# daisy9542/yolo-puncture

Hardware: AMD Instinct MI355X
Metric: images/sec (higher is better)
Workload: dtype bf16

## Files before the change

include/yolop.h:

```cpp
#ifndef YOLOP_H
#define YOLOP_H

#include <stddef.h>
#include <stdint.h>

#ifdef __cplusplus
extern "C" {
#endif

#define YP_OK 0
#define YP_ERR_ARG -1
#define YP_ERR_STATE -2
#define YP_ERR_HIP -3
#define YP_ERR_WEIGHT -4

#define YP_BF16 0
#define YP_F32 1

#define YP_TASK_DETECT 0
#define YP_TASK_SEGMENT 1

#define YP_NM 32
#define YP_MAX_MASKS 480
#define YP_ID_MASKS_FRAMES_BUDGET (1ull << 30)
// ... 137 lines not shown

int yp_debug_force_conv_cfg(int cfg);
int yp_debug_op_cfg(const yp_engine* e, int i, int* cfg);
int yp_debug_last_store_form(void);
int yp_debug_max_workgroups(int n);
int yp_debug_conv_families(int* base, int* num_cfgs, int cap);
int yp_debug_ablation(int v);
int yp_debug_head_clocks(uint64_t* out8);
int yp_debug_attention(const void* qkv_dev, void* o_dev, int dtype, int B, int N, int nh, int kd, int hd, int q_stride, int q_coff, int o_stride,
                       int o_coff, int wgs, int* kernel_out, void* stream);
int yp_debug_attention_form(const void* qkv_dev, void* o_dev, int dtype, int B, int N, int nh, int kd, int hd, int q_stride, int q_coff, int o_stride,
                            int o_coff, int wgs, int form, int* kernel_out, void* stream);
int yp_debug_conv_s2(const void* x_dev, const void* w_dev, const float* bias_dev, const void* res_dev, void* y_dev, int out_f32, int B, int H,
                     int W, int Cin, int Cout, int silu, int cfg, int lds_weights, int64_t* lds_out, char* kernel_out, int kernel_cap,
                     void* stream);
int yp_debug_topk_anchors(const uint32_t* const mk_dev[3], int B, const int hw[3][2], int k, int32_t* sel_out_dev, uint32_t* thr_out_dev, void* stream);
int yp_debug_head_branch_clocks(uint64_t* out8);
int yp_debug_head_winners(yp_engine* e, int32_t* sel_host, float* box_host, float* coeff_host);
int yp_debug_contour_clocks(uint64_t* out12);
int yp_debug_pwsp_clocks(uint64_t* out32);

int yp_tuning_source(const yp_engine* e);

int yp_debug_host_selftest(yp_engine* e);
int yp_debug_graph_info(const yp_engine* e, int64_t* out6);
int yp_debug_head_positions(yp_engine* e, int64_t* out6);
int yp_debug_marker(void* stream);

int yp_set_graph(yp_engine* e, int enable);

// ... 5 lines not shown
```

yolo-puncture_amd/csrc/common.h:

```cpp
#pragma once
#include <hip/hip_runtime.h>
#include <stdint.h>
#include <atomic>
#include <cstdlib>
#include <initializer_list>
#include <string>
#include <type_traits>
#include <vector>

namespace yp {

enum DType { DT_BF16 = 0, DT_F32 = 1 };
enum Act { ACT_NONE = 0, ACT_SILU = 1, ACT_RELU = 2 };

enum OpKind {
    OP_STEM = 0,
    OP_CONV = 1,
    OP_DWCONV = 2,
    OP_POOL5 = 3,
    OP_UPSAMPLE = 4,
    OP_ATTN = 5,
    OP_HEAD = 6,
    OP_CONVT = 7,
    OP_AMAX = 9,
// ... 352 lines not shown
                           size_t rows, hipStream_t st);
hipError_t launch_anchor_max_level(const float* cls, int B, int HW, int nc, unsigned* out, hipStream_t st);

struct DwPwParams {
    const void* x; int x_stride, x_coff; int B, H, W, C; size_t x_bytes;
    const void* w_dw; const float* b_dw; int act_dw;
    const void* w_pw; int Kpad; size_t wpw_bytes; const float* b_pw; int act_pw;
    void* y; int y_stride, y_coff; size_t y_bytes; int Cout; int out_f32;
    unsigned long long* clk;
    int wide;
    const void* w3; int Kpad3; size_t w3_bytes; const float* b3; int C3;
    float* y3; int y3_stride, y3_coff; size_t y3_bytes;
    unsigned* keys;
};
bool dwpw_stream_valid(const DwPwParams& p);
hipError_t launch_dwpw_stream(const DwPwParams& p, hipStream_t st);
struct PwSpParams {
    const void* x; int x_stride, x_coff; size_t x_bytes; int B, H, W, K;
    const void* w1; const float* bias1; int act1, Kpad1, C1; size_t w1_bytes;
    void* y1; int y1_stride, y1_coff;
    const void* res1; int res1_stride, res1_coff;
    int sp;
    int sp_c0, Csp;
    const void* wd; const float* biasd; int actd;
    const void* res; int res_stride, res_coff;
    void* y2; int y2_stride, y2_coff;
    int dbg;
    int wide;
};
bool pwsp_valid(const PwSpParams& p);
// ... 76 lines not shown
```

yolo-puncture_amd/csrc/conv_dwpw.hip:

```cpp
#include "common.h"
#include <cstdio>
#include <cstdlib>
#include <vector>

namespace yp {

template <int TH, int BN, bool OUT_F32, int NW, bool TAIL = false>
__global__ __launch_bounds__(NW * 64) void conv_dwpw_kernel(const DwPwParams p, const int tiles_h, const int tiles_w, const int ntiles,
                                                       const int G) {
    constexpr int WGM = 2, WGN = NW / 2;
    constexpr int RPW = TH / NW;
    static_assert(RPW * NW == TH && RPW >= 1, "rows per wave");
    constexpr int BM = TH * 16;
    constexpr int HP = (TH + 2) * 18;
    constexpr int H_INSTR = (HP * 4 + 63) / 64;
    constexpr int LH = (H_INSTR + NW - 1) / NW;
    constexpr int HB = H_INSTR * 1024;
    constexpr int NSH = 3;
    constexpr int WM = BM / WGM, WN = BN / WGN, FM = WM / 16, FN = WN / 16;
    constexpr int S = FM * FN;
    static_assert(LH + 2 * S < 64, "vmcnt immediate");

    extern __shared__ __attribute__((aligned(1024))) unsigned char smem[];
    const int nchunk = p.C >> 5;
// ... 355 lines not shown
    if (dwpw_stream_valid(p)) return true;
    if ((p.C % 32) != 0 || p.Kpad != p.C || (p.Cout & 3) || (p.y_stride & 3) || (p.y_coff & 3)) return false;
    if (p.x_bytes >= (1ull << 31) || p.y_bytes >= (1ull << 31) || p.wpw_bytes >= (1ull << 31)) return false;
    if ((long)((p.H + 7) / 8 * 8) * ((p.W + 15) / 16 * 16) * 2 > (long)p.H * p.W * 3) return false;
    const int bn = dwpw_bn(p);
    if (bn == 0) return false;
    if ((p.Cout + bn - 1) / bn > 2) return false;
    if (dwpw_tail(p)) {
        if (p.Cout > bn || p.C < 64 || p.C3 <= 0 || p.C3 > 128 || (p.C3 & 3) || (p.y3_stride & 3) || (p.y3_coff & 3) || !p.y3 || !p.b3) return false;
        if (p.Kpad3 != (p.Cout + 31) / 32 * 32 || p.y3_bytes >= (1ull << 31) || p.w3_bytes >= (1ull << 31) || (size_t)p.B * p.H * p.W * 4 >= (1ull << 31)) return false;
    }
    return true;
}

const char* conv_dwpw_kernel_name(const DwPwParams& p) {
    if (dwpw_stream_valid(p)) return "conv_dwpw_stream_kernel";
    const int bn = dwpw_bn(p);
    if (dwpw_tail(p)) return bn == 128 ? "conv_dwpw_kernel<8,128,tail,8>" : "conv_dwpw_kernel<8,64,tail,8>";
    if (p.out_f32) return bn == 128 ? "conv_dwpw_kernel<8,128,true,8>" : "conv_dwpw_kernel<8,64,true,8>";
    return bn == 128 ? "conv_dwpw_kernel<8,128,false,8>" : "conv_dwpw_kernel<8,64,false,8>";
}

template <int BN, bool OUT_F32, bool TAIL = false>
static hipError_t launch_dwpw_t(const DwPwParams& p, hipStream_t st) {
    constexpr int TH = 8, NW = 8;
    const size_t sh = dwpw_lds(TH, BN, p.C, TAIL ? p.C3 : 0);
    const int tiles_h = (p.H + TH - 1) / TH, tiles_w = (p.W + 15) / 16, ntiles = (p.Cout + BN - 1) / BN;
    const int num_tiles = p.B * tiles_h * tiles_w;
    int G = 256 / ntiles;
    if (sh <= 80 * 1024 && NW == 4) G *= 2;
    if (G < 1) G = 1;
// ... 41 lines not shown
```

yolo-puncture_amd/csrc/conv_dwpw_stream.hip:

```cpp
#include "common.h"
#include <cstdlib>

namespace yp {

constexpr int DS_TH = 8, DS_TW = 16;
constexpr int DS_C = 128;
constexpr int DS_HP = (DS_TH + 2) * (DS_TW + 2);
constexpr int DS_PIECES = 48;
constexpr int DS_HB = DS_PIECES * 1024;
constexpr int DS_AB = DS_TH * DS_TW * 256;

template <int NW>
__global__ __launch_bounds__(NW * 64, 2) void conv_dwpw_stream_kernel(const DwPwParams p, const int tiles_h, const int tiles_w, const int num_tiles, const int G) {
    constexpr int RPW = DS_TH / NW;
    constexpr int NFW = 8 / NW;
    constexpr int NSLOT = NW == 8 ? 2 : 1;
    constexpr int NST = DS_TH * NFW;
    extern __shared__ __attribute__((aligned(1024))) unsigned char smem[];
    unsigned char* const Hs = smem;
    unsigned char* const As = smem + NSLOT * DS_HB;
    const int tid = threadIdx.x, lane = tid & 63;
    const int wave = __builtin_amdgcn_readfirstlane(tid >> 6);
    const int fr = lane & 15, fc = lane >> 4;
    const bool wide = NFW % 2 == 0 && p.wide != 0;

    const __amdgpu_buffer_rsrc_t xrs = __builtin_amdgcn_make_buffer_rsrc((void*)p.x, 0, (int)p.x_bytes, 0x00020000);
    const __amdgpu_buffer_rsrc_t wrs = __builtin_amdgcn_make_buffer_rsrc((void*)p.w_pw, 0, (int)p.wpw_bytes, 0x00020000);
    const __amdgpu_buffer_rsrc_t yrs = __builtin_amdgcn_make_buffer_rsrc((void*)p.y, 0, (int)p.y_bytes, 0x00020000);

    unsigned hyx[DS_PIECES / NW];
#pragma unroll
    for (int j = 0; j < DS_PIECES / NW; ++j) {
        const int hp = ((wave + j * NW) * 64 + lane) >> 4;
        const int hy = hp / (DS_TW + 2);
        hyx[j] = (unsigned)((hy << 8) | (hp - hy * (DS_TW + 2)));
    }
    auto issue_tile = [&](int tile, int slot) {
        int t = tile;
        const int tw = t % tiles_w; t /= tiles_w;
        const int th = t % tiles_h;
        const int b = t / tiles_h;
        const int h0 = th * DS_TH - 1, w0 = tw * DS_TW - 1;
        unsigned char* const dst = Hs + slot * DS_HB;
#pragma unroll
        for (int j = 0; j < DS_PIECES / NW; ++j) {
            const int ii = wave + j * NW;
            const int s = ii * 64 + lane;
            const int hp = s >> 4, c = s & 15;
            unsigned q = hyx[j];
            asm volatile("" : "+v"(q));
            const int hy = (int)(q >> 8), hx = (int)(q & 255u);
            const int hi = h0 + hy, wi = w0 + hx;
            const bool ok = tile < num_tiles && hp < DS_HP && (unsigned)hi < (unsigned)p.H && (unsigned)wi < (unsigned)p.W;
            const unsigned voff = ok ? (unsigned)((((b * p.H + hi) * p.W + wi) * p.x_stride + p.x_coff + c * 8) * 2) : kBufferOOB;
            __builtin_amdgcn_raw_ptr_buffer_load_lds(xrs, (lds_void*)(dst + ii * 1024), 16, voff, 0, 0, 0);
        }
    };
    int tile = blockIdx.x;
    issue_tile(tile, 0);

    f32x2 wd[9], bd;
    {
        const unsigned* w32 = (const unsigned*)p.w_dw;
#pragma unroll
        for (int t = 0; t < 9; ++t) {
            const unsigned u = w32[t * (DS_C / 2) + lane];
// ... 2 lines not shown
        bd = f32x2{p.b_dw[2 * lane], p.b_dw[2 * lane + 1]};
    }
    bf16x8 wreg[4][NFW];
    float bpw[NFW][4];
#pragma unroll
    for (int i = 0; i < NFW; ++i) {
#pragma unroll
        for (int ks = 0; ks < 4; ++ks) {
            const unsigned voff = (unsigned)((weight_row_channel((wave * NFW + i) * 16 + fr, wide) * p.Kpad + (ks >> 1) * 64 + fc * 16 + (ks & 1) * 8) * 2);
            const __attribute__((ext_vector_type(4))) unsigned v = __builtin_amdgcn_raw_buffer_load_b128(wrs, voff, 0, 0);
            wreg[ks][i] = __builtin_bit_cast(bf16x8, v);
        }
#pragma unroll
        for (int r = 0; r < 4; ++r) { const int co = wave * NFW * 16 + acc_channel(i, fc, wide) + r; bpw[i][r] = (co < p.Cout) ? p.b_pw[co] : 0.f; }
    }
    wait_vmcnt<0>();
#pragma unroll
    for (int t = 0; t < 9; ++t) asm volatile("" : "+v"(wd[t]));
    asm volatile("" : "+v"(bd));
#pragma unroll
    for (int i = 0; i < NFW; ++i) {
#pragma unroll
        for (int ks = 0; ks < 4; ++ks) asm volatile("" : "+v"(wreg[ks][i]));
#pragma unroll
        for (int r = 0; r < 4; ++r) asm volatile("" : "+v"(bpw[i][r]));
    }

    const unsigned as_l = lds_addr(As);
    for (int it = 0; tile < num_tiles; tile += G, ++it) {
        if (it == 0) wait_vmcnt<0>();
        else if (wide) wait_vmcnt<NST / 2>();
        else wait_vmcnt<NST>();
        __builtin_amdgcn_s_barrier();
        const int slot = NSLOT == 2 ? (it & 1) : 0;
        if (NSLOT == 2) issue_tile(tile + G, slot ^ 1);
        int t = tile;
        const int tw = t % tiles_w; t /= tiles_w;
        const int th = t % tiles_h;
        const int b = t / tiles_h;
#pragma unroll
        for (int rr = 0; rr < RPW; ++rr) {
            const int row = wave * RPW + rr;
            f32x2 win[3][3];
            auto rd = [&](int ky, int col) -> f32x2 {
                const unsigned u = *(const unsigned*)(Hs + slot * DS_HB + ((row + ky) * (DS_TW + 2) + col) * 256 + lane * 4);
                return f32x2{__uint_as_float(u << 16), __uint_as_float(u & 0xffff0000u)};
            };
#pragma unroll
            for (int ky = 0; ky < 3; ++ky) { win[ky][0] = rd(ky, 0); win[ky][1] = rd(ky, 1); }
#pragma unroll
            for (int x = 0; x < DS_TW; ++x) {
#pragma unroll
                for (int ky = 0; ky < 3; ++ky) win[ky][2] = rd(ky, x + 2);
                f32x2 a = bd;
#pragma unroll
                for (int ky = 0; ky < 3; ++ky)
#pragma unroll
                    for (int kx = 0; kx < 3; ++kx) a = __builtin_elementwise_fma(win[ky][kx], wd[ky * 3 + kx], a);
                if (p.act_dw == ACT_SILU) {
                    f32x2 e = a * -1.4426950408889634f;
                    e[0] = __builtin_amdgcn_exp2f(e[0]); e[1] = __builtin_amdgcn_exp2f(e[1]);
                    e = e + 1.0f;
                    e[0] = __builtin_amdgcn_rcpf(e[0]); e[1] = __builtin_amdgcn_rcpf(e[1]);
                    a = a * e;
                }
                __attribute__((aligned(4))) __bf16 o[2] = {(__bf16)a[0], (__bf16)a[1]};
                const int px = row * DS_TW + x;
                const unsigned dst = as_l + (unsigned)(px * 256 + (((lane >> 2) ^ (px & 15)) << 4) + (lane & 3) * 4);
                asm volatile("ds_write_b32 %0, %1" : : "v"(dst), "v"(*(const unsigned*)o) : "memory");
#pragma unroll
                for (int ky = 0; ky < 3; ++ky) { win[ky][0] = win[ky][1]; win[ky][1] = win[ky][2]; }
            }
        }
        asm volatile("s_waitcnt lgkmcnt(0)" ::: "memory");
        __builtin_amdgcn_s_barrier();
        if (NSLOT == 1) issue_tile(tile + G, 0);
        f32x4 acc[NFW][DS_TH];
#pragma unroll
        for (int i = 0; i < NFW; ++i)
#pragma unroll
            for (int f = 0; f < DS_TH; ++f) acc[i][f] = f32x4{bpw[i][0], bpw[i][1], bpw[i][2], bpw[i][3]};
#pragma unroll
        for (int ks = 0; ks < 4; ++ks) {
            const int ch = (ks >> 1) * 8 + fc * 2 + (ks & 1);
            bf16x8 xf[DS_TH];
#pragma unroll
            for (int f = 0; f < DS_TH; ++f) xf[f] = *(const bf16x8*)(As + (f * 16 + fr) * 256 + ((ch ^ fr) << 4));
#pragma unroll
            for (int i = 0; i < NFW; ++i)
#pragma unroll
                for (int f = 0; f < DS_TH; ++f) acc[i][f] = __builtin_amdgcn_mfma_f32_16x16x32_bf16(wreg[ks][i], xf[f], acc[i][f], 0, 0, 0);
        }
        const int wo = tw * DS_TW + fr;
        if (wide) {
#pragma unroll
            for (int j = 0; j < NFW / 2; ++j) {
                const int co = wave * NFW * 16 + acc_channel(2 * j, fc, true);
#pragma unroll
                for (int f = 0; f < DS_TH; ++f) {
                    const int ho = th * DS_TH + f;
                    const bool ok = ho < p.H && wo < p.W;
                    float v[2][4];
#pragma unroll
                    for (int h = 0; h < 2; ++h) {
#pragma unroll
                        for (int q = 0; q < 4; ++q) v[h][q] = acc[2 * j + h][f][q];
                        if (p.act_pw == ACT_SILU) silu4_packed(v[h]);
                    }
                    store_bf16x8(v[0], v[1], yrs, ok ? (unsigned)((((b * p.H + ho) * p.W + wo) * p.y_stride + p.y_coff + co) * 2) : kBufferOOB);
                }
            }
            continue;
        }
#pragma unroll
        for (int i = 0; i < NFW; ++i) {
            const int co = (wave * NFW + i) * 16 + fc * 4;
#pragma unroll
            for (int f = 0; f < DS_TH; ++f) {
                const int ho = th * DS_TH + f;
                const bool ok = ho < p.H && wo < p.W && co < p.Cout;
                float v[4] = {acc[i][f][0], acc[i][f][1], acc[i][f][2], acc[i][f][3]};
                if (p.act_pw == ACT_SILU) silu4_packed(v);
                const unsigned off = ok ? (unsigned)((((b * p.H + ho) * p.W + wo) * p.y_stride + p.y_coff + co) * 2) : kBufferOOB;
                store_bf16x4(v, yrs, off);
            }
        }
    }
    wait_vmcnt<0>();
}

bool dwpw_stream_valid(const DwPwParams& p) {
    static const bool off = env_on("YOLOP_NO_DWPW_STREAM");
    if (off || p.w3 || p.out_f32 || p.clk) return false;
    if (p.C != DS_C || p.Kpad != DS_C || p.Cout != 128) return false;
    if ((p.x_stride & 7) || (p.x_coff & 7) || (p.y_stride & 3) || (p.y_coff & 3)) return false;
    if (p.x_bytes >= (1ull << 31) || p.y_bytes >= (1ull << 31) || p.wpw_bytes >= (1ull << 31)) return false;
    if (p.act_dw != ACT_SILU && p.act_dw != ACT_NONE) return false;
    if (p.act_pw != ACT_SILU && p.act_pw != ACT_NONE) return false;
    return (long)((p.H + DS_TH - 1) / DS_TH * DS_TH) * ((p.W + DS_TW - 1) / DS_TW * DS_TW) * 2 <= (long)p.H * p.W * 3;
}

template <int NW>
static hipError_t launch_dwpw_stream_t(const DwPwParams& p_in, hipStream_t st) {
    DwPwParams p = p_in;
    p.wide = wide_store_ok(p_in.wide, 8 / NW, p_in.Cout, p_in.y_stride, p_in.y_coff, p_in.out_f32 != 0) ? 1 : 0;
    const size_t sh = (size_t)(NW == 8 ? 2 : 1) * DS_HB + DS_AB;
    auto kern = conv_dwpw_stream_kernel<NW>;
    static size_t granted = 0;
    if (hipError_t e = allow_dynamic_lds((const void*)kern, sh, granted)) return e;
    const int tiles_h = (p.H + DS_TH - 1) / DS_TH, tiles_w = (p.W + DS_TW - 1) / DS_TW;
    const int num_tiles = p.B * tiles_h * tiles_w;
    const int gmax = NW == 8 ? 256 : 512;
    int G = num_tiles < gmax ? num_tiles : gmax;
    if (const int cap = debug_max_workgroups()) G = G < cap ? G : cap;
    hipLaunchKernelGGL(kern, dim3((unsigned)G), dim3(NW * 64), sh, st, p, tiles_h, tiles_w, num_tiles, G);
    return hipGetLastError();
}

hipError_t launch_dwpw_stream(const DwPwParams& p, hipStream_t st) {
    if (!dwpw_stream_valid(p)) return hipErrorInvalidValue;
    static const bool one = env_on("YOLOP_DWPW_STREAM_ONE");
    return one ? launch_dwpw_stream_t<8>(p, st) : launch_dwpw_stream_t<4>(p, st);
}

}
```

yolo-puncture_amd/csrc/engine.hip:

```cpp
#include "../../include/yolop.h"
#include "common.h"
#include <algorithm>
#include <array>
#include <chrono>

#include <cmath>
#include <cstdarg>
#include <cstdio>
#include <cstring>
#include <cstdlib>
#include <dlfcn.h>
#include <fcntl.h>
#include <fstream>
#include <map>
#include <sstream>
#include <memory>

using namespace yp;

static thread_local char g_err[512] = "";
static int fail(int code, const char* fmt, ...) {
    va_list ap;
    va_start(ap, fmt);
    vsnprintf(g_err, sizeof(g_err), fmt, ap);
// ... 806 lines not shown
    int (*absorbed)(const yp_engine& e, const Op& o, int m[3]);
    std::string (*admit)(const yp_engine& e, const Op& o, int& cfg);
    void (*views)(const yp_engine& e, const Op& o, View& in, View& extra);
    hipError_t (*launch)(const yp_engine& e, const Op& o, const RunArgs& a, hipStream_t st);
};
static int link1(int i, int m[3]) { m[0] = i; return i >= 0 ? 1 : 0; }

static int dwpw_absorbed(const yp_engine&, const Op& o, int m[3]) { return link1(o.fuse_dw, m); }
static std::string dwpw_admit(const yp_engine& e, const Op& o, int&) {
    const DwPwParams q = dwpw_params(e, o);
    return conv_dwpw_valid(q) ? conv_dwpw_kernel_name(q) : "";
}
static void dwpw_views(const yp_engine& e, const Op& o, View& in, View&) { in = e.ops[o.fuse_dw].in; }
static hipError_t dwpw_launch(const yp_engine& e, const Op& o, const RunArgs&, hipStream_t st) { return launch_conv_dwpw(dwpw_params(e, o), st); }

static int tail_absorbed(const yp_engine& e, const Op& o, int m[3]) {
    if (o.fuse_tail < 0) return 0;
    m[0] = e.ops[o.fuse_tail].fuse_dw; m[1] = o.fuse_tail; m[2] = o.tail_amax;
    return o.tail_amax >= 0 ? 3 : 2;
}
static std::string tail_admit(const yp_engine& e, const Op& o, int& cfg) {
    return e.tail && e.ops[o.fuse_tail].form == FORM_DWPW ? dwpw_admit(e, o, cfg) : "";
}
static void tail_views(const yp_engine& e, const Op& o, View& in, View& extra) {
    in = e.ops[e.ops[o.fuse_tail].fuse_dw].in;
    if (o.tail_amax >= 0) extra = e.ops[o.tail_amax].out;
}

static int s2pw_absorbed(const yp_engine&, const Op& o, int m[3]) { return link1(o.fuse_pre, m); }
static std::string s2pw_admit(const yp_engine& e, const Op& o, int& cfg) {
    const ConvParams q = conv_params(e, o);
    const int c = conv_halo_s2_pw_cfg(q);
    if (c < 0) return "";
    cfg = conv_halo_s2_family.base + c;
    return conv_halo_s2_family.symbol(q, c);
}
static void s2pw_views(const yp_engine& e, const Op& o, View& in, View&) { in = e.ops[o.fuse_pre].in; }
// ... 1551 lines not shown
    const int before = conv_halo_s2_lds_weights(lds_weights ? 1 : 0);
    const bool ok = f.valid(p, cfg - f.base);
    hipError_t err = hipSuccess;
    if (lds_out) *lds_out = (int64_t)conv_halo_s2_lds_bytes(p, cfg - f.base);
    if (ok && kernel_out && kernel_cap > 0) std::snprintf(kernel_out, (size_t)kernel_cap, "%s", f.symbol(p, cfg - f.base).c_str());
    if (ok && !host_only) {
        hipStream_t st = (hipStream_t)stream;
        err = f.launch(p, cfg - f.base, st);
        if (err == hipSuccess) err = hipStreamSynchronize(st);
    }
    conv_halo_s2_lds_weights(before);
    if (!ok)
        return fail(YP_ERR_ARG, "yp_debug_conv_s2: configuration %d does not admit B %d, H %d, W %d, Cin %d, Cout %d%s%s%s", cfg, B, H, W, Cin, Cout,
                    res_dev ? ", residual" : "", out_f32 ? ", fp32 output" : "", lds_weights ? ", weights in LDS" : "");
    if (err != hipSuccess) return fail(YP_ERR_HIP, "yp_debug_conv_s2: %s", hipGetErrorString(err));
    return YP_OK;
}

int yp_tuning_source(const yp_engine* e) {
    if (!e) return YP_ERR_ARG;
    return e->tune_source;
}

int yp_debug_graph_info(const yp_engine* e, int64_t* out6) {
    if (!e || !out6) return fail(YP_ERR_ARG, "yp_debug_graph_info: null argument");
    out6[0] = e->n_captures; out6[1] = e->g_nodes; out6[2] = e->g_edges; out6[3] = e->g_edges_expected;
    out6[4] = (int64_t)e->lanes_used.size() + 1; out6[5] = e->gexec ? 1 : 0;
    return YP_OK;
}

// ... 446 lines not shown
```

yolo-puncture_amd/engine.py:

```python
from __future__ import annotations

import ctypes as C
import os
from typing import Dict, List, Optional, Tuple

import numpy as np
import torch

from .weights import fold_state

_LIB: Optional[C.CDLL] = None
_HERE = os.path.dirname(os.path.abspath(__file__))
LIB_PATH = os.environ.get("YOLOP_LIB") or os.path.join(_HERE, "libyolop.so")

YP_BF16, YP_F32 = 0, 1
TASK_DETECT, TASK_SEGMENT = 0, 1
OP_KINDS = {0: "stem", 1: "conv", 2: "dwconv", 3: "pool5", 4: "upsample", 5: "attn", 6: "head", 7: "convT", 8: "pool3", 9: "amax"}
FORMS = ("plain", "dwpw", "dwpw_tail", "s2pw", "frontend", "c2f", "scdown", "pwsp", "cls_out")


class ModelDesc(C.Structure):
    _fields_ = [("variant", C.c_int), ("nc", C.c_int), ("task", C.c_int), ("dtype", C.c_int), ("max_det", C.c_int), ("family", C.c_int)]


# ... 31 lines not shown
    lib.yp_mask_contours_large_workspace.restype = C.c_size_t
    lib.yp_mask_contours_large.argtypes = [vp, C.c_int, C.c_int, C.c_int, C.c_int, C.c_int, vp, vp, vp, C.c_int, vp, C.c_int, C.c_int, C.c_int, vp,
                                           C.c_size_t, vp]
    lib.yp_mask_contours_large.restype = C.c_int
    lib.yp_plan.argtypes = [vp, C.c_int, C.c_int, C.c_int]
    lib.yp_max_batch.argtypes = [vp, C.c_int, C.c_int]
    lib.yp_max_batch.restype = C.c_int
    lib.yp_debug_topk_anchors.argtypes = [C.POINTER(vp), C.c_int, C.POINTER(C.c_int), C.c_int, vp, vp, vp]
    lib.yp_debug_topk_anchors.restype = C.c_int
    lib.yp_debug_attention.argtypes = [vp, vp] + [C.c_int] * 11 + [ip, vp]
    lib.yp_debug_attention.restype = C.c_int
    lib.yp_debug_attention_form.argtypes = [vp, vp] + [C.c_int] * 12 + [ip, vp]
    lib.yp_debug_attention_form.restype = C.c_int
    lib.yp_debug_conv_s2.argtypes = [vp, vp, vp, vp, vp] + [C.c_int] * 9 + [C.POINTER(C.c_int64), C.c_char_p, C.c_int, vp]
    lib.yp_debug_conv_s2.restype = C.c_int
    lib.yp_set_attention_form.argtypes = [vp, C.c_int]
    lib.yp_set_attention_form.restype = C.c_int
    lib.yp_op_info.argtypes = [vp, C.c_int, C.c_char_p, C.c_int, ip, C.POINTER(C.c_double), C.POINTER(C.c_double)]
    lib.yp_op_output.argtypes = [vp, C.c_int, ip, ip, ip]
    lib.yp_op_kernel.argtypes = [vp, C.c_int, C.c_char_p, C.c_int]
    lib.yp_op_fusion.argtypes = [vp, C.c_int, ip, ip]
    lib.yp_op_fusion.restype = C.c_int
    lib.yp_debug_op_form.argtypes = [vp, C.c_int, ip, ip, C.c_int]
    lib.yp_debug_op_form.restype = C.c_int
    lib.yp_run_op.argtypes = [vp, C.c_int, vp, vp, vp, vp, vp]
    lib.yp_tensor_write.argtypes = [vp, C.c_int, C.c_int, C.c_int, vp]
    lib.yp_tensor_count.argtypes = [vp]
    lib.yp_tensor_info.argtypes = [vp, C.c_int, C.c_char_p, C.c_int, ip, ip]
    lib.yp_tensor_read.argtypes = [vp, C.c_int, vp]
    lib.yp_profile.argtypes = [vp, vp, C.c_int, C.c_int, C.c_int, vp, vp, vp, vp, C.c_int, vp]
# ... 44 lines not shown
    for fn in ("yp_comm_unique_id", "yp_comm_create", "yp_allgather", "yp_comm_destroy"):
        getattr(lib, fn).restype = C.c_int
    for fn in ("yp_create", "yp_destroy", "yp_weight_count", "yp_weight_info", "yp_set_weight", "yp_finalize",
               "yp_forward", "yp_proto", "yp_masks", "yp_plan", "yp_op_info", "yp_op_output", "yp_op_input", "yp_tensor_count",
               "yp_tensor_info", "yp_tensor_read", "yp_profile", "yp_set_graph", "yp_run_op", "yp_tensor_write",
               "yp_op_kernel", "yp_set_autotune", "yp_debug_force_conv_cfg", "yp_debug_ablation"):
        getattr(lib, fn).restype = C.c_int
    if path is None:
        _LIB = lib
    return lib


EXPORTS = ["yp_last_error", "yp_create", "yp_destroy", "yp_weight_count", "yp_weight_info", "yp_set_weight",
           "yp_finalize", "yp_forward", "yp_proto", "yp_masks", "yp_id_mask_resized", "yp_plan", "yp_op_info", "yp_op_output", "yp_op_input", "yp_op_fusion",
           "yp_tensor_count", "yp_tensor_info", "yp_tensor_read", "yp_profile", "yp_set_graph", "yp_run_op",
           "yp_tensor_write", "yp_op_kernel", "yp_set_autotune", "yp_tuning_export", "yp_tuning_import", "yp_set_nms", "yp_debug_force_conv_cfg", "yp_debug_op_cfg", "yp_debug_op_form", "yp_debug_last_store_form", "yp_debug_max_workgroups", "yp_debug_conv_families", "yp_debug_ablation", "yp_debug_head_clocks", "yp_debug_head_branch_clocks", "yp_debug_head_winners", "yp_debug_contour_clocks", "yp_debug_pwsp_clocks", "yp_debug_host_selftest", "yp_debug_graph_info", "yp_tuning_source", "yp_debug_head_positions", "yp_debug_marker", "yp_max_batch", "yp_debug_topk_anchors", "yp_debug_attention", "yp_debug_attention_form", "yp_debug_conv_s2", "yp_set_attention_form", "yp_letterbox", "yp_letterbox_batch", "yp_masks_frames", "yp_masks_frames_input", "yp_id_masks_frames", "yp_id_masks_frames_workspace", "yp_mask_contours",
           "yp_mask_contours_scaled", "yp_mask_contours_large_workspace", "yp_mask_contours_large", "yp_comm_unique_id", "yp_comm_create", "yp_allgather", "yp_comm_destroy",
           "yp_u2net_create", "yp_u2net_destroy", "yp_u2net_weight_count", "yp_u2net_weight_info", "yp_u2net_set_weight", "yp_u2net_finalize",
           "yp_u2net_forward", "yp_u2net_forward_crops", "yp_u2net_set_graph", "yp_u2net_tensor_count", "yp_u2net_tensor_info", "yp_u2net_tensor_read",
           "yp_u2net_op_count", "yp_u2net_op_info",
           "yp_cls_create", "yp_cls_destroy", "yp_cls_weight_count", "yp_cls_weight_info", "yp_cls_set_weight", "yp_cls_finalize",
           "yp_cls_forward", "yp_cls_set_graph", "yp_cls_tensor_count", "yp_cls_tensor_info", "yp_cls_tensor_read"]


MAX_ANCHORS = 294912
MAX_MASKS = 480
ID_MASKS_FRAMES_BUDGET = 1 << 30
ATTENTION_FORMS = {"auto": 0, "stream": 1, "stream_wide": 3}


def _attention_form(form) -> int:
# ... 58 lines not shown
                              C.c_void_p(res.data_ptr()) if res is not None else None, C.c_void_p(y.data_ptr()), int(bool(out_f32)), B, H, W, Cin, Cout,
                              int(bool(silu)), int(cfg), int(bool(lds_weights)), None, None, 0, C.c_void_p(_stream_ptr(x.device)))
    if rc < 0:
        raise YolopError(lib.yp_last_error().decode())
    return y


def conv_s2_admits(cfg: int, B: int, H: int, W: int, Cin: int, Cout: int, res: bool = False, out_f32: bool = False,
                   lds_weights: bool = False) -> Tuple[bool, int, str]:
    lib = load_library()
    lds = C.c_int64(0)
    name = C.create_string_buffer(160)
    rc = lib.yp_debug_conv_s2(None, None, None, C.c_void_p(1) if res else None, None, int(bool(out_f32)), int(B), int(H), int(W), int(Cin), int(Cout),
                              1, int(cfg), int(bool(lds_weights)), C.byref(lds), name, 160, None)
    return rc >= 0, int(lds.value), name.value.decode()


def conv_families() -> List[Tuple[int, int]]:
    lib = load_library()
    n = lib.yp_debug_conv_families(None, None, 0)
    base, num = (C.c_int * n)(), (C.c_int * n)()
    lib.yp_debug_conv_families(base, num, n)
    return list(zip(base, num))


def _stream_ptr(device: torch.device) -> int:
    return int(torch.cuda.current_stream(device).cuda_stream)


def letterbox_device(src: torch.Tensor, geo: dict, out: Optional[torch.Tensor] = None, pad_value: int = 114) -> torch.Tensor:
# ... 447 lines not shown
```

Before: 23320.

## Fuse class-logit tail GEMM and key sigmoid into streaming dw-pw kernel

Adds a TAIL variant to the streaming depthwise+pointwise kernel. The pointwise output is written back to LDS and a third small GEMM (class logits, up to 80 channels) is run in-kernel, along with the per-pixel max-sigmoid key, so the mid tensor no longer makes a global round trip and a separate cls_out launch is avoided. This routes head cls branches with w3 set through the stream kernel instead of the older tiled tail kernel. In exchange it adds extra barriers, holds more registers for the w3 weights, and moves the pointwise GEMM into smaller passes.

```diff
diff --git a/include/yolop.h b/include/yolop.h
--- a/include/yolop.h
+++ b/include/yolop.h
@@ -175,6 +175,9 @@
 int yp_debug_conv_s2(const void* x_dev, const void* w_dev, const float* bias_dev, const void* res_dev, void* y_dev, int out_f32, int B, int H,
                      int W, int Cin, int Cout, int silu, int cfg, int lds_weights, int64_t* lds_out, char* kernel_out, int kernel_cap,
                      void* stream);
+int yp_debug_dwpw_tail(const void* x_dev, const void* w_dw_dev, const float* b_dw_dev, const void* w_pw_dev, const float* b_pw_dev, const void* w3_dev,
+                       const float* b3_dev, void* mid_dev, float* logits_dev, uint32_t* keys_dev, int B, int H, int W, int nc, int y_stride, int y_coff,
+                       int act_dw, int act_pw, int fused, void* stream);
 int yp_debug_topk_anchors(const uint32_t* const mk_dev[3], int B, const int hw[3][2], int k, int32_t* sel_out_dev, uint32_t* thr_out_dev, void* stream);
 int yp_debug_head_branch_clocks(uint64_t* out8);
 int yp_debug_head_winners(yp_engine* e, int32_t* sel_host, float* box_host, float* coeff_host);
diff --git a/yolo-puncture_amd/csrc/common.h b/yolo-puncture_amd/csrc/common.h
--- a/yolo-puncture_amd/csrc/common.h
+++ b/yolo-puncture_amd/csrc/common.h
@@ -390,6 +390,9 @@
     unsigned* keys;
 };
 bool dwpw_stream_valid(const DwPwParams& p);
+bool dwpw_stream_tail_valid(const DwPwParams& p);
+const char* dwpw_stream_kernel_name(const DwPwParams& p);
+int dwpw_stream_tiles(const DwPwParams& p);
 hipError_t launch_dwpw_stream(const DwPwParams& p, hipStream_t st);
 struct PwSpParams {
     const void* x; int x_stride, x_coff; size_t x_bytes; int B, H, W, K;
diff --git a/yolo-puncture_amd/csrc/conv_dwpw.hip b/yolo-puncture_amd/csrc/conv_dwpw.hip
--- a/yolo-puncture_amd/csrc/conv_dwpw.hip
+++ b/yolo-puncture_amd/csrc/conv_dwpw.hip
@@ -393,7 +393,7 @@
 }
 
 const char* conv_dwpw_kernel_name(const DwPwParams& p) {
-    if (dwpw_stream_valid(p)) return "conv_dwpw_stream_kernel";
+    if (dwpw_stream_valid(p)) return dwpw_stream_kernel_name(p);
     const int bn = dwpw_bn(p);
     if (dwpw_tail(p)) return bn == 128 ? "conv_dwpw_kernel<8,128,tail,8>" : "conv_dwpw_kernel<8,64,tail,8>";
     if (p.out_f32) return bn == 128 ? "conv_dwpw_kernel<8,128,true,8>" : "conv_dwpw_kernel<8,64,true,8>";
diff --git a/yolo-puncture_amd/csrc/conv_dwpw_stream.hip b/yolo-puncture_amd/csrc/conv_dwpw_stream.hip
--- a/yolo-puncture_amd/csrc/conv_dwpw_stream.hip
+++ b/yolo-puncture_amd/csrc/conv_dwpw_stream.hip
@@ -10,23 +10,25 @@
 constexpr int DS_HB = DS_PIECES * 1024;
 constexpr int DS_AB = DS_TH * DS_TW * 256;
 
-template <int NW>
+template <int NW, int NF3>
 __global__ __launch_bounds__(NW * 64, 2) void conv_dwpw_stream_kernel(const DwPwParams p, const int tiles_h, const int tiles_w, const int num_tiles, const int G) {
     constexpr int RPW = DS_TH / NW;
     constexpr int NFW = 8 / NW;
     constexpr int NSLOT = NW == 8 ? 2 : 1;
-    constexpr int NST = DS_TH * NFW;
+    constexpr bool TAIL = NF3 > 0;
+    constexpr int NST = TAIL ? RPW * (NF3 + 1) : DS_TH * NFW;
     extern __shared__ __attribute__((aligned(1024))) unsigned char smem[];
     unsigned char* const Hs = smem;
     unsigned char* const As = smem + NSLOT * DS_HB;
     const int tid = threadIdx.x, lane = tid & 63;
     const int wave = __builtin_amdgcn_readfirstlane(tid >> 6);
     const int fr = lane & 15, fc = lane >> 4;
-    const bool wide = NFW % 2 == 0 && p.wide != 0;
+    const bool wide = !TAIL && NFW % 2 == 0 && p.wide != 0;
 
     const __amdgpu_buffer_rsrc_t xrs = __builtin_amdgcn_make_buffer_rsrc((void*)p.x, 0, (int)p.x_bytes, 0x00020000);
     const __amdgpu_buffer_rsrc_t wrs = __builtin_amdgcn_make_buffer_rsrc((void*)p.w_pw, 0, (int)p.wpw_bytes, 0x00020000);
-    const __amdgpu_buffer_rsrc_t yrs = __builtin_amdgcn_make_buffer_rsrc((void*)p.y, 0, (int)p.y_bytes, 0x00020000);
+    const __amdgpu_buffer_rsrc_t yrs = __builtin_amdgcn_make_buffer_rsrc(TAIL ? (void*)p.y3 : p.y, 0, (int)(TAIL ? p.y3_bytes : p.y_bytes), 0x00020000);
+    const __amdgpu_buffer_rsrc_t krs = __builtin_amdgcn_make_buffer_rsrc((TAIL && p.keys) ? (void*)p.keys : p.y, 0, (int)((TAIL && p.keys) ? (size_t)p.B * p.H * p.W * 4 : p.y_bytes), 0x00020000);
 
     unsigned hyx[DS_PIECES / NW];
 #pragma unroll
@@ -47,9 +49,18 @@
             const int ii = wave + j * NW;
             const int s = ii * 64 + lane;
             const int hp = s >> 4, c = s & 15;
-            unsigned q = hyx[j];
-            asm volatile("" : "+v"(q));
-            const int hy = (int)(q >> 8), hx = (int)(q & 255u);
+            int hy, hx;
+            if (TAIL) {
+                int g = fc;
+                asm volatile("" : "+v"(g));
+                const int hq = ii * 4 + g;
+                hy = (hq * 57) >> 10;
+                hx = hq - hy * (DS_TW + 2);
+            } else {
+                unsigned q = hyx[j];
+                asm volatile("" : "+v"(q));
+                hy = (int)(q >> 8); hx = (int)(q & 255u);
+            }
             const int hi = h0 + hy, wi = w0 + hx;
             const bool ok = tile < num_tiles && hp < DS_HP && (unsigned)hi < (unsigned)p.H && (unsigned)wi < (unsigned)p.W;
             const unsigned voff = ok ? (unsigned)((((b * p.H + hi) * p.W + wi) * p.x_stride + p.x_coff + c * 8) * 2) : kBufferOOB;
@@ -82,7 +93,31 @@
 #pragma unroll
         for (int r = 0; r < 4; ++r) { const int co = wave * NFW * 16 + acc_channel(i, fc, wide) + r; bpw[i][r] = (co < p.Cout) ? p.b_pw[co] : 0.f; }
     }
+    constexpr int NF3A = TAIL ? NF3 : 1;
+    bf16x8 w3reg[4][NF3A];
+    float b3[NF3A];
+    if (TAIL) {
+        const __amdgpu_buffer_rsrc_t w3rs = __builtin_amdgcn_make_buffer_rsrc((void*)p.w3, 0, (int)p.w3_bytes, 0x00020000);
+#pragma unroll
+        for (int a = 0; a < NF3A; ++a) {
+#pragma unroll
+            for (int ks = 0; ks < 4; ++ks) {
+                const unsigned voff = (unsigned)(((a * 16 + fr) * p.Kpad3 + ks * 32 + fc * 8) * 2);
+                const __attribute__((ext_vector_type(4))) unsigned v = __builtin_amdgcn_raw_buffer_load_b128(w3rs, voff, 0, 0);
+                w3reg[ks][a] = __builtin_bit_cast(bf16x8, v);
+            }
+            b3[a] = (a * 16 + fr < p.C3) ? p.b3[a * 16 + fr] : 0.f;
+        }
+    }
     wait_vmcnt<0>();
+    if (TAIL) {
+#pragma unroll
+        for (int a = 0; a < NF3A; ++a) {
+#pragma unroll
+            for (int ks = 0; ks < 4; ++ks) asm volatile("" : "+v"(w3reg[ks][a]));
+            asm volatile("" : "+v"(b3[a]));
+        }
+    }
 #pragma unroll
     for (int t = 0; t < 9; ++t) asm volatile("" : "+v"(wd[t]));
     asm volatile("" : "+v"(bd));
@@ -96,6 +131,9 @@
 
     const unsigned as_l = lds_addr(As);
     for (int it = 0; tile < num_tiles; tile += G, ++it) {
+        int ln = lane;
+        if (TAIL) asm volatile("" : "+v"(ln));
+        const int lr = ln & 15, lc = ln >> 4;
         if (it == 0) wait_vmcnt<0>();
         else if (wide) wait_vmcnt<NST / 2>();
         else wait_vmcnt<NST>();
@@ -111,7 +149,7 @@
             const int row = wave * RPW + rr;
             f32x2 win[3][3];
             auto rd = [&](int ky, int col) -> f32x2 {
-                const unsigned u = *(const unsigned*)(Hs + slot * DS_HB + ((row + ky) * (DS_TW + 2) + col) * 256 + lane * 4);
+                const unsigned u = *(const unsigned*)(Hs + slot * DS_HB + ((row + ky) * (DS_TW + 2) + col) * 256 + ln * 4);
                 return f32x2{__uint_as_float(u << 16), __uint_as_float(u & 0xffff0000u)};
             };
 #pragma unroll
@@ -134,7 +172,7 @@
                 }
                 __attribute__((aligned(4))) __bf16 o[2] = {(__bf16)a[0], (__bf16)a[1]};
                 const int px = row * DS_TW + x;
-                const unsigned dst = as_l + (unsigned)(px * 256 + (((lane >> 2) ^ (px & 15)) << 4) + (lane & 3) * 4);
+                const unsigned dst = as_l + (unsigned)(px * 256 + (((ln >> 2) ^ (px & 15)) << 4) + (ln & 3) * 4);
                 asm volatile("ds_write_b32 %0, %1" : : "v"(dst), "v"(*(const unsigned*)o) : "memory");
 #pragma unroll
                 for (int ky = 0; ky < 3; ++ky) { win[ky][0] = win[ky][1]; win[ky][1] = win[ky][2]; }
@@ -143,6 +181,79 @@
         asm volatile("s_waitcnt lgkmcnt(0)" ::: "memory");
         __builtin_amdgcn_s_barrier();
         if (NSLOT == 1) issue_tile(tile + G, 0);
+        if constexpr (TAIL) {
+            constexpr int PF = NW == 4 ? 2 : 4, NPS = DS_TH / PF;
+            u32x2 pk[NFW][DS_TH];
+#pragma unroll
+            for (int h = 0; h < NPS; ++h) {
+                f32x4 acc[NFW][PF];
+#pragma unroll
+                for (int i = 0; i < NFW; ++i)
+#pragma unroll
+                    for (int f = 0; f < PF; ++f) acc[i][f] = f32x4{bpw[i][0], bpw[i][1], bpw[i][2], bpw[i][3]};
+#pragma unroll
+                for (int ks = 0; ks < 4; ++ks) {
+                    const int ch = (ks >> 1) * 8 + lc * 2 + (ks & 1);
+                    bf16x8 xf[PF];
+#pragma unroll
+                    for (int f = 0; f < PF; ++f) xf[f] = *(const bf16x8*)(As + ((h * (PF) + f) * 16 + lr) * 256 + ((ch ^ lr) << 4));
+#pragma unroll
+                    for (int i = 0; i < NFW; ++i)
+#pragma unroll
+                        for (int f = 0; f < PF; ++f) acc[i][f] = __builtin_amdgcn_mfma_f32_16x16x32_bf16(wreg[ks][i], xf[f], acc[i][f], 0, 0, 0);
+                }
+#pragma unroll
+                for (int i = 0; i < NFW; ++i)
+#pragma unroll
+                    for (int f = 0; f < PF; ++f) {
+                        float v[4] = {acc[i][f][0], acc[i][f][1], acc[i][f][2], acc[i][f][3]};
+                        if (p.act_pw == ACT_SILU) silu4_packed(v);
+                        pk[i][h * (PF) + f] = pack_bf16x4(v);
+                    }
+            }
+            __builtin_amdgcn_s_barrier();
+#pragma unroll
+            for (int i = 0; i < NFW; ++i) {
+                const int q = (wave * NFW + i) * 2 + (lc >> 1);
+#pragma unroll
+                for (int f = 0; f < DS_TH; ++f) {
+                    const unsigned dst = as_l + (unsigned)((f * 16 + lr) * 256 + ((q ^ lr) << 4) + (lc & 1) * 8);
+                    asm volatile("ds_write_b64 %0, %1" : : "v"(dst), "v"(pk[i][f]) : "memory");
+                }
+            }
+            asm volatile("s_waitcnt lgkmcnt(0)" ::: "memory");
+            __builtin_amdgcn_s_barrier();
+            const int wo = tw * DS_TW + lr;
+#pragma unroll
+            for (int rr = 0; rr < RPW; ++rr) {
+                const int row = wave * RPW + rr;
+                f32x4 a3[NF3A];
+#pragma unroll
+                for (int a = 0; a < NF3A; ++a) a3[a] = f32x4{__shfl(b3[a], lc * 4, 64), __shfl(b3[a], lc * 4 + 1, 64), __shfl(b3[a], lc * 4 + 2, 64), __shfl(b3[a], lc * 4 + 3, 64)};
+#pragma unroll
+                for (int ks = 0; ks < 4; ++ks) {
+                    const bf16x8 xf = *(const bf16x8*)(As + (row * 16 + lr) * 256 + (((ks * 4 + lc) ^ lr) << 4));
+#pragma unroll
+                    for (int a = 0; a < NF3A; ++a) a3[a] = __builtin_amdgcn_mfma_f32_16x16x32_bf16(w3reg[ks][a], xf, a3[a], 0, 0, 0);
+                }
+                const int ho = th * DS_TH + row;
+                const bool ok = ho < p.H && wo < p.W;
+                const unsigned m = (unsigned)((b * p.H + ho) * p.W + wo);
+                float mx = -INFINITY;
+#pragma unroll
+                for (int a = 0; a < NF3A; ++a) {
+                    const int co = a * 16 + lc * 4;
+                    const bool in = co < p.C3;
+                    if (in) mx = fmaxf(mx, fmaxf(fmaxf(a3[a][0], a3[a][1]), fmaxf(a3[a][2], a3[a][3])));
+                    const float v[4] = {a3[a][0], a3[a][1], a3[a][2], a3[a][3]};
+                    store_f32x4(v, yrs, (ok && in) ? (m * (unsigned)p.y3_stride + (unsigned)(p.y3_coff + co)) * 4u : kBufferOOB);
+                }
+                mx = fmaxf(mx, __shfl_xor(mx, 16, 64));
+                mx = fmaxf(mx, __shfl_xor(mx, 32, 64));
+                __builtin_amdgcn_raw_buffer_store_b32(__float_as_uint(sigmoid_ieee(mx)), krs, (p.keys && ok && lc == 0) ? m * 4u : kBufferOOB, 0, 0);
+            }
+            continue;
+        }
         f32x4 acc[NFW][DS_TH];
 #pragma unroll
         for (int i = 0; i < NFW; ++i)
@@ -150,20 +261,20 @@
             for (int f = 0; f < DS_TH; ++f) acc[i][f] = f32x4{bpw[i][0], bpw[i][1], bpw[i][2], bpw[i][3]};
 #pragma unroll
         for (int ks = 0; ks < 4; ++ks) {
-            const int ch = (ks >> 1) * 8 + fc * 2 + (ks & 1);
+            const int ch = (ks >> 1) * 8 + lc * 2 + (ks & 1);
             bf16x8 xf[DS_TH];
 #pragma unroll
-            for (int f = 0; f < DS_TH; ++f) xf[f] = *(const bf16x8*)(As + (f * 16 + fr) * 256 + ((ch ^ fr) << 4));
+            for (int f = 0; f < DS_TH; ++f) xf[f] = *(const bf16x8*)(As + (f * 16 + lr) * 256 + ((ch ^ lr) << 4));
 #pragma unroll
             for (int i = 0; i < NFW; ++i)
 #pragma unroll
                 for (int f = 0; f < DS_TH; ++f) acc[i][f] = __builtin_amdgcn_mfma_f32_16x16x32_bf16(wreg[ks][i], xf[f], acc[i][f], 0, 0, 0);
         }
-        const int wo = tw * DS_TW + fr;
+        const int wo = tw * DS_TW + lr;
         if (wide) {
 #pragma unroll
             for (int j = 0; j < NFW / 2; ++j) {
-                const int co = wave * NFW * 16 + acc_channel(2 * j, fc, true);
+                const int co = wave * NFW * 16 + acc_channel(2 * j, lc, true);
 #pragma unroll
                 for (int f = 0; f < DS_TH; ++f) {
                     const int ho = th * DS_TH + f;
@@ -182,7 +293,7 @@
         }
 #pragma unroll
         for (int i = 0; i < NFW; ++i) {
-            const int co = (wave * NFW + i) * 16 + fc * 4;
+            const int co = (wave * NFW + i) * 16 + lc * 4;
 #pragma unroll
             for (int f = 0; f < DS_TH; ++f) {
                 const int ho = th * DS_TH + f;
@@ -197,9 +308,10 @@
     wait_vmcnt<0>();
 }
 
-bool dwpw_stream_valid(const DwPwParams& p) {
-    static const bool off = env_on("YOLOP_NO_DWPW_STREAM");
-    if (off || p.w3 || p.out_f32 || p.clk) return false;
+static int dwpw_stream_nf3(const DwPwParams& p) { return p.C3 <= 16 ? 1 : 5; }
+
+static bool dwpw_stream_shape_ok(const DwPwParams& p) {
+    if (p.out_f32 || p.clk) return false;
     if (p.C != DS_C || p.Kpad != DS_C || p.Cout != 128) return false;
     if ((p.x_stride & 7) || (p.x_coff & 7) || (p.y_stride & 3) || (p.y_coff & 3)) return false;
     if (p.x_bytes >= (1ull << 31) || p.y_bytes >= (1ull << 31) || p.wpw_bytes >= (1ull << 31)) return false;
@@ -208,12 +320,36 @@
     return (long)((p.H + DS_TH - 1) / DS_TH * DS_TH) * ((p.W + DS_TW - 1) / DS_TW * DS_TW) * 2 <= (long)p.H * p.W * 3;
 }
 
-template <int NW>
+bool dwpw_stream_tail_valid(const DwPwParams& p) {
+    if (!p.w3 || !p.b3 || !p.y3 || !dwpw_stream_shape_ok(p)) return false;
+    if (p.C3 < 4 || p.C3 > 80 || (p.C3 & 3) || p.Kpad3 != DS_C || (p.y3_stride & 3) || (p.y3_coff & 3)) return false;
+    if (p.w3_bytes < (size_t)dwpw_stream_nf3(p) * 16 * DS_C * 2) return false;
+    return p.y3_bytes < (1ull << 31) && p.w3_bytes < (1ull << 31) && (size_t)p.B * p.H * p.W * 4 < (1ull << 31);
+}
+
+bool dwpw_stream_valid(const DwPwParams& p) {
+    static const bool off = env_on("YOLOP_NO_DWPW_STREAM");
+    static const bool off_tail = env_on("YOLOP_NO_STREAM_TAIL");
+    if (off) return false;
+    return p.w3 ? (!off_tail && dwpw_stream_tail_valid(p)) : dwpw_stream_shape_ok(p);
+}
+
+int dwpw_stream_tiles(const DwPwParams& p) { return p.B * ((p.H + DS_TH - 1) / DS_TH) * ((p.W + DS_TW - 1) / DS_TW); }
+
+static bool dwpw_stream_one() { static const bool one = env_on("YOLOP_DWPW_STREAM_ONE"); return one; }
+
+const char* dwpw_stream_kernel_name(const DwPwParams& p) {
+    if (!p.w3) return "conv_dwpw_stream_kernel";
+    if (dwpw_stream_one()) return dwpw_stream_nf3(p) == 1 ? "conv_dwpw_stream_kernel<8,tail,1>" : "conv_dwpw_stream_kernel<8,tail,5>";
+    return dwpw_stream_nf3(p) == 1 ? "conv_dwpw_stream_kernel<4,tail,1>" : "conv_dwpw_stream_kernel<4,tail,5>";
+}
+
+template <int NW, int NF3>
 static hipError_t launch_dwpw_stream_t(const DwPwParams& p_in, hipStream_t st) {
     DwPwParams p = p_in;
     p.wide = wide_store_ok(p_in.wide, 8 / NW, p_in.Cout, p_in.y_stride, p_in.y_coff, p_in.out_f32 != 0) ? 1 : 0;
     const size_t sh = (size_t)(NW == 8 ? 2 : 1) * DS_HB + DS_AB;
-    auto kern = conv_dwpw_stream_kernel<NW>;
+    auto kern = conv_dwpw_stream_kernel<NW, NF3>;
     static size_t granted = 0;
     if (hipError_t e = allow_dynamic_lds((const void*)kern, sh, granted)) return e;
     const int tiles_h = (p.H + DS_TH - 1) / DS_TH, tiles_w = (p.W + DS_TW - 1) / DS_TW;
@@ -226,9 +362,13 @@
 }
 
 hipError_t launch_dwpw_stream(const DwPwParams& p, hipStream_t st) {
-    if (!dwpw_stream_valid(p)) return hipErrorInvalidValue;
-    static const bool one = env_on("YOLOP_DWPW_STREAM_ONE");
-    return one ? launch_dwpw_stream_t<8>(p, st) : launch_dwpw_stream_t<4>(p, st);
-}
-
-}
+    if (p.w3 ? !dwpw_stream_tail_valid(p) : !dwpw_stream_valid(p)) return hipErrorInvalidValue;
+    const bool one = dwpw_stream_one();
+    if (p.w3) {
+        if (dwpw_stream_nf3(p) == 1) return one ? launch_dwpw_stream_t<8, 1>(p, st) : launch_dwpw_stream_t<4, 1>(p, st);
+        return one ? launch_dwpw_stream_t<8, 5>(p, st) : launch_dwpw_stream_t<4, 5>(p, st);
+    }
+    return one ? launch_dwpw_stream_t<8, 0>(p, st) : launch_dwpw_stream_t<4, 0>(p, st);
+}
+
+}
diff --git a/yolo-puncture_amd/csrc/engine.hip b/yolo-puncture_amd/csrc/engine.hip
--- a/yolo-puncture_amd/csrc/engine.hip
+++ b/yolo-puncture_amd/csrc/engine.hip
@@ -844,13 +844,19 @@
 static void dwpw_views(const yp_engine& e, const Op& o, View& in, View&) { in = e.ops[o.fuse_dw].in; }
 static hipError_t dwpw_launch(const yp_engine& e, const Op& o, const RunArgs&, hipStream_t st) { return launch_conv_dwpw(dwpw_params(e, o), st); }
 
+constexpr int TAIL_MIN_TILES = 256;
 static int tail_absorbed(const yp_engine& e, const Op& o, int m[3]) {
     if (o.fuse_tail < 0) return 0;
     m[0] = e.ops[o.fuse_tail].fuse_dw; m[1] = o.fuse_tail; m[2] = o.tail_amax;
     return o.tail_amax >= 0 ? 3 : 2;
 }
 static std::string tail_admit(const yp_engine& e, const Op& o, int& cfg) {
-    return e.tail && e.ops[o.fuse_tail].form == FORM_DWPW ? dwpw_admit(e, o, cfg) : "";
+    const Op& pw = e.ops[o.fuse_tail];
+    if (pw.form != FORM_DWPW) return "";
+    if (e.tail) return dwpw_admit(e, o, cfg);
+    const DwPwParams q = dwpw_params(e, o);
+    if (!dwpw_stream_valid(dwpw_params(e, pw)) || !dwpw_stream_valid(q) || dwpw_stream_tiles(q) < TAIL_MIN_TILES) return "";
+    return dwpw_stream_kernel_name(q);
 }
 static void tail_views(const yp_engine& e, const Op& o, View& in, View& extra) {
     in = e.ops[e.ops[o.fuse_tail].fuse_dw].in;
@@ -2432,6 +2438,41 @@
         return fail(YP_ERR_ARG, "yp_debug_conv_s2: configuration %d does not admit B %d, H %d, W %d, Cin %d, Cout %d%s%s%s", cfg, B, H, W, Cin, Cout,
                     res_dev ? ", residual" : "", out_f32 ? ", fp32 output" : "", lds_weights ? ", weights in LDS" : "");
     if (err != hipSuccess) return fail(YP_ERR_HIP, "yp_debug_conv_s2: %s", hipGetErrorString(err));
+    return YP_OK;
+}
+
+int yp_debug_dwpw_tail(const void* x_dev, const void* w_dw_dev, const float* b_dw_dev, const void* w_pw_dev, const float* b_pw_dev, const void* w3_dev,
+                       const float* b3_dev, void* mid_dev, float* logits_dev, uint32_t* keys_dev, int B, int H, int W, int nc, int y_stride, int y_coff,
+                       int act_dw, int act_pw, int fused, void* stream) {
+    const bool host_only = !x_dev && !w_dw_dev && !b_dw_dev && !w_pw_dev && !b_pw_dev && !w3_dev && !b3_dev && !mid_dev && !logits_dev && !keys_dev;
+    if (!host_only && (!x_dev || !w_dw_dev || !b_dw_dev || !w_pw_dev || !b_pw_dev || !w3_dev || !b3_dev || !logits_dev || !keys_dev || (!fused && !mid_dev)))
+        return fail(YP_ERR_ARG, "yp_debug_dwpw_tail: null argument");
+    if (B < 1 || H < 1 || W < 1 || nc < 1 || y_stride < 1 || y_coff < 0 || (int64_t)y_coff + nc > y_stride)
+        return fail(YP_ERR_ARG, "yp_debug_dwpw_tail: bad size (B %d, H %d, W %d, nc %d, y_stride %d, y_coff %d)", B, H, W, nc, y_stride, y_coff);
+    const size_t px = (size_t)B * H * W;
+    const void* const one = (const void*)1;
+    DwPwParams p{};
+    p.x = host_only ? one : x_dev; p.x_stride = 128; p.x_coff = 0; p.B = B; p.H = H; p.W = W; p.C = 128; p.x_bytes = px * 128 * 2;
+    p.w_dw = w_dw_dev; p.b_dw = b_dw_dev; p.act_dw = act_dw ? ACT_SILU : ACT_NONE;
+    p.w_pw = w_pw_dev; p.Kpad = 128; p.wpw_bytes = (size_t)128 * 128 * 2; p.b_pw = b_pw_dev; p.act_pw = act_pw ? ACT_SILU : ACT_NONE;
+    p.y = mid_dev; p.y_stride = 128; p.y_coff = 0; p.y_bytes = px * 128 * 2; p.Cout = 128; p.out_f32 = 0;
+    p.wide = 1;
+    DwPwParams t = p;
+    t.w3 = host_only ? one : w3_dev; t.Kpad3 = 128; t.w3_bytes = (size_t)128 * 128 * 2; t.b3 = host_only ? (const float*)one : b3_dev; t.C3 = nc;
+    t.y3 = host_only ? (float*)one : logits_dev; t.y3_stride = y_stride; t.y3_coff = y_coff; t.y3_bytes = px * (size_t)y_stride * 4;
+    t.keys = keys_dev;
+    ClsOutParams c{};
+    c.x = mid_dev; c.x_stride = 128; c.x_coff = 0; c.x_bytes = p.y_bytes;
+    c.M = (int)px; c.K = 128; c.nc = nc; c.w = w3_dev; c.Kpad = 128; c.w_bytes = t.w3_bytes; c.bias = b3_dev;
+    c.y = logits_dev; c.y_stride = y_stride; c.y_coff = y_coff; c.keys = keys_dev;
+    if (px * 128 * 2 >= (1ull << 31) || !dwpw_stream_tail_valid(t) || !cls_out_valid(c))
+        return fail(YP_ERR_ARG, "yp_debug_dwpw_tail: the streaming kernel's TAIL form does not admit B %d, H %d, W %d, nc %d, y_stride %d, y_coff %d", B, H, W, nc, y_stride, y_coff);
+    if (host_only) return YP_OK;
+    hipStream_t st = (hipStream_t)stream;
+    hipError_t err = fused ? launch_dwpw_stream(t, st) : launch_dwpw_stream(p, st);
+    if (err == hipSuccess && !fused) err = launch_cls_out(c, st);
+    if (err == hipSuccess) err = hipStreamSynchronize(st);
+    if (err != hipSuccess) return fail(YP_ERR_HIP, "yp_debug_dwpw_tail: %s", hipGetErrorString(err));
     return YP_OK;
 }
 
diff --git a/yolo-puncture_amd/engine.py b/yolo-puncture_amd/engine.py
--- a/yolo-puncture_amd/engine.py
+++ b/yolo-puncture_amd/engine.py
@@ -69,6 +69,8 @@
     lib.yp_debug_attention_form.restype = C.c_int
     lib.yp_debug_conv_s2.argtypes = [vp, vp, vp, vp, vp] + [C.c_int] * 9 + [C.POINTER(C.c_int64), C.c_char_p, C.c_int, vp]
     lib.yp_debug_conv_s2.restype = C.c_int
+    lib.yp_debug_dwpw_tail.argtypes = [vp] * 10 + [C.c_int] * 9 + [vp]
+    lib.yp_debug_dwpw_tail.restype = C.c_int
     lib.yp_set_attention_form.argtypes = [vp, C.c_int]
     lib.yp_set_attention_form.restype = C.c_int
     lib.yp_op_info.argtypes = [vp, C.c_int, C.c_char_p, C.c_int, ip, C.POINTER(C.c_double), C.POINTER(C.c_double)]
@@ -143,7 +145,7 @@
 EXPORTS = ["yp_last_error", "yp_create", "yp_destroy", "yp_weight_count", "yp_weight_info", "yp_set_weight",
            "yp_finalize", "yp_forward", "yp_proto", "yp_masks", "yp_id_mask_resized", "yp_plan", "yp_op_info", "yp_op_output", "yp_op_input", "yp_op_fusion",
            "yp_tensor_count", "yp_tensor_info", "yp_tensor_read", "yp_profile", "yp_set_graph", "yp_run_op",
-           "yp_tensor_write", "yp_op_kernel", "yp_set_autotune", "yp_tuning_export", "yp_tuning_import", "yp_set_nms", "yp_debug_force_conv_cfg", "yp_debug_op_cfg", "yp_debug_op_form", "yp_debug_last_store_form", "yp_debug_max_workgroups", "yp_debug_conv_families", "yp_debug_ablation", "yp_debug_head_clocks", "yp_debug_head_branch_clocks", "yp_debug_head_winners", "yp_debug_contour_clocks", "yp_debug_pwsp_clocks", "yp_debug_host_selftest", "yp_debug_graph_info", "yp_tuning_source", "yp_debug_head_positions", "yp_debug_marker", "yp_max_batch", "yp_debug_topk_anchors", "yp_debug_attention", "yp_debug_attention_form", "yp_debug_conv_s2", "yp_set_attention_form", "yp_letterbox", "yp_letterbox_batch", "yp_masks_frames", "yp_masks_frames_input", "yp_id_masks_frames", "yp_id_masks_frames_workspace", "yp_mask_contours",
+           "yp_tensor_write", "yp_op_kernel", "yp_set_autotune", "yp_tuning_export", "yp_tuning_import", "yp_set_nms", "yp_debug_force_conv_cfg", "yp_debug_op_cfg", "yp_debug_op_form", "yp_debug_last_store_form", "yp_debug_max_workgroups", "yp_debug_conv_families", "yp_debug_ablation", "yp_debug_head_clocks", "yp_debug_head_branch_clocks", "yp_debug_head_winners", "yp_debug_contour_clocks", "yp_debug_pwsp_clocks", "yp_debug_host_selftest", "yp_debug_graph_info", "yp_tuning_source", "yp_debug_head_positions", "yp_debug_marker", "yp_max_batch", "yp_debug_topk_anchors", "yp_debug_attention", "yp_debug_attention_form", "yp_debug_conv_s2", "yp_debug_dwpw_tail", "yp_set_attention_form", "yp_letterbox", "yp_letterbox_batch", "yp_masks_frames", "yp_masks_frames_input", "yp_id_masks_frames", "yp_id_masks_frames_workspace", "yp_mask_contours",
            "yp_mask_contours_scaled", "yp_mask_contours_large_workspace", "yp_mask_contours_large", "yp_comm_unique_id", "yp_comm_create", "yp_allgather", "yp_comm_destroy",
            "yp_u2net_create", "yp_u2net_destroy", "yp_u2net_weight_count", "yp_u2net_weight_info", "yp_u2net_set_weight", "yp_u2net_finalize",
            "yp_u2net_forward", "yp_u2net_forward_crops", "yp_u2net_set_graph", "yp_u2net_tensor_count", "yp_u2net_tensor_info", "yp_u2net_tensor_read",
@@ -232,6 +234,42 @@
     rc = lib.yp_debug_conv_s2(None, None, None, C.c_void_p(1) if res else None, None, int(bool(out_f32)), int(B), int(H), int(W), int(Cin), int(Cout),
                               1, int(cfg), int(bool(lds_weights)), C.byref(lds), name, 160, None)
     return rc >= 0, int(lds.value), name.value.decode()
+
+
+def dwpw_tail(x: torch.Tensor, w_dw: torch.Tensor, b_dw: torch.Tensor, w_pw: torch.Tensor, b_pw: torch.Tensor, w3: torch.Tensor, b3: torch.Tensor,
+              fused: bool, act_dw: bool = True, act_pw: bool = True, y_stride: Optional[int] = None, y_coff: int = 0) -> Tuple[torch.Tensor, torch.Tensor]:
+    lib = load_library()
+    if x.dim() != 4 or x.shape[3] != 128 or x.dtype != torch.bfloat16 or not x.is_cuda or not x.is_contiguous():
+        raise ValueError("x: contiguous device bf16 [B, H, W, 128]")
+    B, H, W, _ = (int(v) for v in x.shape)
+    nc = int(w3.shape[0])
+    if tuple(w_dw.shape) != (128, 3, 3) or tuple(w_pw.shape) != (128, 128) or tuple(w3.shape) != (nc, 128) or nc > 128 or \
+            any(t.dtype != torch.bfloat16 for t in (w_dw, w_pw, w3)):
+        raise ValueError("w_dw: bf16 [128, 3, 3], w_pw: bf16 [128, 128], w3: bf16 [nc, 128]")
+    if tuple(b_dw.shape) != (128,) or tuple(b_pw.shape) != (128,) or tuple(b3.shape) != (nc,) or any(t.dtype != torch.float32 for t in (b_dw, b_pw, b3)):
+        raise ValueError("b_dw, b_pw: float32 [128], b3: float32 [nc]")
+    if not all(t.device == x.device for t in (w_dw, b_dw, w_pw, b_pw, w3, b3)):
+        raise ValueError("all tensors on x's device")
+    y_stride = nc if y_stride is None else int(y_stride)
+    wd = w_dw.permute(1, 2, 0).reshape(9, 128).contiguous()
+    w3p = torch.zeros((128, 128), dtype=torch.bfloat16, device=x.device)
+    w3p[:nc] = w3
+    mid = None if fused else torch.empty((B, H, W, 128), dtype=torch.bfloat16, device=x.device)
+    logits = torch.zeros((B, H, W, y_stride), dtype=torch.float32, device=x.device)
+    keys = torch.zeros((B, H, W), dtype=torch.int32, device=x.device)
+    ptr = lambda t: C.c_void_p(t.data_ptr())
+    rc = lib.yp_debug_dwpw_tail(ptr(x), ptr(wd), ptr(b_dw.contiguous()), ptr(w_pw.contiguous()), ptr(b_pw.contiguous()), ptr(w3p), ptr(b3.contiguous()),
+                                ptr(mid) if mid is not None else None, ptr(logits), ptr(keys), B, H, W, nc, y_stride, int(y_coff),
+                                int(bool(act_dw)), int(bool(act_pw)), int(bool(fused)), C.c_void_p(_stream_ptr(x.device)))
+    if rc < 0:
+        raise YolopError(lib.yp_last_error().decode())
+    return logits, keys
+
+
+def dwpw_tail_admits(B: int, H: int, W: int, nc: int, y_stride: Optional[int] = None, y_coff: int = 0) -> bool:
+    lib = load_library()
+    rc = lib.yp_debug_dwpw_tail(*([None] * 10), int(B), int(H), int(W), int(nc), int(nc if y_stride is None else y_stride), int(y_coff), 1, 1, 1, None)
+    return rc >= 0
 
 
 def conv_families() -> List[Tuple[int, int]]:
```

Result: faster. 23560 (median of 6 runs) (+1.1%).
